# CUG-EMI/HMCMT2D

Measured on NVIDIA B200. Metric: leapfrog_steps_per_sec, higher is better.
Workload: dtype f64 (complex128)

## Files before the change

hmcmt2d_b200/csrc/hmcmt_b200.cu:

```cuda
#include <dlfcn.h>
#include <nccl.h>

#include <algorithm>
#include <cmath>
#include <cstdlib>
#include <cstring>
#include <new>
#include <vector>

#include "../../include/hmcmt_b200.h"
#include "band_factor.cuh"
#include "band_solve.cuh"
#include "mf_solver.cuh"
#include "mt_kernels.cuh"

using namespace hmcmt;

namespace {

template <typename Tp>
struct DevBuf {
    Tp* p = nullptr;
    size_t n = 0;
    int alloc(size_t count) {
// ... 154 lines not shown
        case 14: return launch_factor_T<14>(st, sys, nsys, dom, fwdJobs);
        default: return kErrArg;
    }
}
int launch_solve(cudaStream_t st, int T, const SolveJob* jobs, int njobs, const BandDom& dom) {
    switch (T) {
        case 2: return launch_solve_T<2>(st, jobs, njobs, dom);
        case 4: return launch_solve_T<4>(st, jobs, njobs, dom);
        case 6: return launch_solve_T<6>(st, jobs, njobs, dom);
        case 8: return launch_solve_T<8>(st, jobs, njobs, dom);
        case 10: return launch_solve_T<10>(st, jobs, njobs, dom);
        case 12: return launch_solve_T<12>(st, jobs, njobs, dom);
        case 14: return launch_solve_T<14>(st, jobs, njobs, dom);
        default: return kErrArg;
    }
}
int mf_leaf_size() {
    const char* e = std::getenv("HMCMT_MF_LEAF");
    const int v = e ? std::atoi(e) : 16;
    return v < 1 ? 1 : v;
}
int mf_cross_size() {
    const char* e = std::getenv("HMCMT_MF_CROSS");
    const int v = e ? std::atoi(e) : 0;
    return v < 0 ? 0 : v;
}
int mf_push_size() {
    const char* e = std::getenv("HMCMT_MF_PUSH");
    const int v = e ? std::atoi(e) : 2;
    return v < 0 ? 0 : (v > 7 ? 7 : v);
}
int mf_small_front() {
    const char* e = std::getenv("HMCMT_MF_FSMALL");
    int v = e ? std::atoi(e) : 144;
    return v < 0 ? 0 : (v > 144 ? 144 : v);
}
}

namespace {

void linear_interp(double point, const std::vector<double>& x, int& iL, int& iR, double& wL, double& wR) {
    int n = (int)x.size(), ind = 0;
    double best = std::fabs(point - x[0]);
    for (int i = 1; i < n; ++i) {
        double d = std::fabs(point - x[i]);
        if (d < best) { best = d; ind = i; }
    }
    if (point - x[ind] > 0) { iL = ind; iR = ind + 1; } else { iL = ind - 1; iR = ind; }
    iL = std::max(std::min(iL, n - 1), 0);
    iR = std::max(std::min(iR, n - 1), 0);
    if (iL == iR) { wL = 0.5; wR = 0.5; return; }
    double len = x[iR] - x[iL];
    wL = 1 - (point - x[iL]) / len;
    wR = 1 - (x[iR] - point) / len;
}

__global__ void k_pack_pred(int nData, int nFull, const int* __restrict__ packed2full, const cplx* __restrict__ predFull,
                            cplx* __restrict__ out) {
    int i = blockIdx.x * blockDim.x + threadIdx.x, ch = blockIdx.y;
    if (i < nData) out[(size_t)ch * nData + i] = predFull[(size_t)ch * nFull + packed2full[i]];
}
__global__ void k_pack_pred_real(int nData, int nFull, const int* __restrict__ packed2full, const double* __restrict__ respFull,
                                 double* __restrict__ out) {
    int i = blockIdx.x * blockDim.x + threadIdx.x, ch = blockIdx.y;
    if (i < nData) out[(size_t)ch * nData + i] = respFull[(size_t)ch * 2 * nFull + packed2full[i]];
}
__global__ void k_kick_masked(int nAC, double dt, int kstep, const int* __restrict__ L, const double* __restrict__ grad,
                              double* __restrict__ p) {
// ... 1511 lines not shown
```

hmcmt2d_b200/csrc/mf_kernels.cuh:

```cuda
#pragma once
#include "band_factor.cuh"
#include "mf_solver.cuh"

namespace hmcmt {
namespace mf {

__host__ __device__ __forceinline__ size_t kg_off(int ld, int i, int j, int plane) {
    return ((size_t)((j >> 2) * 2 + plane) * ld + i) * 4 + (j & 3);
}

struct Tables {
    const Front* fronts;
    const int* rows;
    const int* rel;
    const int* children;
    const OrigEntry* orig;
    const Chunk* chunks;
    const int* pos2orig;
    double* fac;
    double* arena[2];
    int64_t facStride, arenaStride[2];
    const cplx* vals;
    int64_t valStride;
    int* status;
// ... 16 lines not shown
    f.re[0] = T[lane]; f.re[1] = T[32 + lane]; f.im[0] = T[64 + lane]; f.im[1] = T[96 + lane];
}
__device__ __forceinline__ void frag_load_t(TileFrag& f, const double* T, int g, int t) {
    const int o0 = tl_off(t, g), o1 = tl_off(4 + t, g);
    f.re[0] = T[o0]; f.re[1] = T[o1]; f.im[0] = T[64 + o0]; f.im[1] = T[64 + o1];
}
__device__ __forceinline__ void frag_store(const TileFrag& f, double* T, int lane) {
    T[lane] = f.re[0]; T[32 + lane] = f.re[1]; T[64 + lane] = f.im[0]; T[96 + lane] = f.im[1];
}
__device__ __forceinline__ void cfrag_load(TileFrag& c, const double* T, int g, int t) {
    const int o = tl_off(g, 2 * t);
    const double2 r = *reinterpret_cast<const double2*>(T + o), i = *reinterpret_cast<const double2*>(T + 64 + o);
    c.re[0] = r.x; c.re[1] = r.y; c.im[0] = i.x; c.im[1] = i.y;
}
__device__ __forceinline__ void cfrag_store(const TileFrag& c, double* T, int g, int t, double sign = 1.0) {
    const int o = tl_off(g, 2 * t);
    *reinterpret_cast<double2*>(T + o) = make_double2(sign * c.re[0], sign * c.re[1]);
    *reinterpret_cast<double2*>(T + 64 + o) = make_double2(sign * c.im[0], sign * c.im[1]);
}
__device__ __forceinline__ void frag_mma(TileFrag& c, TileFrag& x, const TileFrag& a, const TileFrag& b) {
#pragma unroll
    for (int kk = 0; kk < 2; ++kk) {
        dmma884(c.re, a.re[kk], b.re[kk]);
        dmma884(c.im, a.re[kk], b.im[kk]);
        dmma884(x.re, -a.im[kk], b.im[kk]);
        dmma884(x.im, a.im[kk], b.re[kk]);
    }
}
__device__ __forceinline__ void frag_zero(TileFrag& c) { c.re[0] = c.re[1] = c.im[0] = c.im[1] = 0.0; }
__device__ __forceinline__ void frag_add(TileFrag& c, const TileFrag& x) {
    c.re[0] += x.re[0]; c.re[1] += x.re[1]; c.im[0] += x.im[0]; c.im[1] += x.im[1];
}

template <int NW, bool PC = false>
__device__ __forceinline__ void mf_front_factor(double* __restrict__ tiles, double* __restrict__ scratch, double* __restrict__ mbuf,
                                                double* __restrict__ nainv, int* __restrict__ fail, const int nb, const int npb,
                                                const int sReal, unsigned long long* __restrict__ prof = nullptr) {
    const int tid = threadIdx.x, lane = tid & 31;
    long long _s0 = prof ? clock64() : 0;
#define MF_SWEEP_MARK(slot) do { if (prof && tid == 0) { const long long _t = clock64(); atomicAdd(prof + (slot), (unsigned long long)(_t - _s0)); _s0 = _t; } } while (0)
    const int warp = __shfl_sync(0xffffffffu, tid >> 5, 0);
    const int g = lane >> 2, t = lane & 3;
    double* const rawb = scratch;
    double* const mmb = scratch + (size_t)npb * 128;
    for (int kb = 0; kb < npb; ++kb) {
        if (warp == 0) {
            const double* D = mf_tile(tiles, kb, kb);
            auto sym = [&](int r, int c, int pl) { return r >= c ? D[pl * 64 + tl_off(r, c)] : D[pl * 64 + tl_off(c, r)]; };
            cplx a0 = mk(sym(g, 2 * t, 0), sym(g, 2 * t, 1)), a1 = mk(sym(g, 2 * t + 1, 0), sym(g, 2 * t + 1, 1));
            bool bad = false;
            const int left = sReal - 8 * kb;
            gj_invert8<(NW > 4)>(a0, a1, bad, g, t, left < 8 ? (left < 0 ? 0 : left) : 8);
            if (__any_sync(0xffffffffu, bad) && lane == 0) *fail = 1;
            TileFrag p;
            p.re[0] = -a0.x; p.re[1] = -a1.x; p.im[0] = -a0.y; p.im[1] = -a1.y;
            cfrag_store(p, nainv, g, t);
            __syncwarp();
            double* Dw = mf_tile(tiles, kb, kb);
            cfrag_store(p, Dw, g, t);
        }
        if (npb == 1) break;
        __syncthreads();
        MF_SWEEP_MARK(0);
        for (int I = warp; I < npb; I += NW) {
            if (I == kb) continue;
            TileFrag a, b, c, x;
            if (I > kb) frag_load(a, mf_tile(tiles, I, kb), lane);
            else frag_load_t(a, mf_tile(tiles, kb, I), g, t);
            frag_load(b, nainv, lane);
            frag_zero(c); frag_zero(x);
// ... 24 lines not shown
                    TileFrag a, b, c, x;
                    frag_load(a, mmb + (size_t)I * 128, lane);
                    frag_load(b, rawb + (size_t)J * 128, lane);
                    cfrag_load(c, T, g, t);
                    frag_zero(x);
                    frag_mma(c, x, a, b);
                    frag_add(c, x);
                    cfrag_store(c, T, g, t);
                }
                J += NW;
                while (J > I) { J -= I + 1; ++I; }
            }
        }
        __syncthreads();
        MF_SWEEP_MARK(1);
    }
    const int nub = nb - npb;
    if (nub == 0) { __syncthreads(); return; }
    __syncthreads();
    if (npb == 1) MF_SWEEP_MARK(0);
    for (int Iu = warp; Iu < nub; Iu += NW) {
        const int I = npb + Iu;
        for (int kb = 0; kb < npb; ++kb) {
            TileFrag c, x;
            frag_zero(c); frag_zero(x);
            for (int j = 0; j < npb; ++j) {
                TileFrag a, b;
                frag_load(a, mf_tile<PC>(tiles, npb, I, j), lane);
                if (kb >= j) frag_load(b, mf_tile(tiles, kb, j), lane);
                else frag_load_t(b, mf_tile(tiles, j, kb), g, t);
                frag_mma(c, x, a, b);
            }
            frag_add(c, x);
            cfrag_store(c, mbuf + (size_t)(Iu * npb + kb) * 128, g, t);
        }
    }
    __syncthreads();
    MF_SWEEP_MARK(2);
    if (PC) return;
    {
        const int nU = nub * (nub + 1) / 2;
        int I = 0, J = warp;
        while (J > I) { J -= I + 1; ++I; }
        constexpr bool kPair = NW > 4;
        for (int L = warp; L < nU; L += (kPair ? 2 : 1) * NW) {
            const int I0 = I, J0 = J;
            J += NW;
            while (J > I) { J -= I + 1; ++I; }
            const bool two = kPair && L + NW < nU;
            const int I1 = I, J1 = J;
            if (kPair) {
                J += NW;
                while (J > I) { J -= I + 1; ++I; }
            }
            double* T0 = mf_tile(tiles, npb + I0, npb + J0);
            double* T1 = mf_tile(tiles, npb + I1, npb + J1);
            TileFrag c0, x0, c1, x1;
            cfrag_load(c0, T0, g, t);
            frag_zero(x0);
            if (two) { cfrag_load(c1, T1, g, t); frag_zero(x1); }
            for (int kb = 0; kb < npb; ++kb) {
                TileFrag a, b;
                frag_load(a, mbuf + (size_t)(I0 * npb + kb) * 128, lane);
                frag_load(b, mf_tile(tiles, npb + J0, kb), lane);
                frag_mma(c0, x0, a, b);
                if (two) {
                    frag_load(a, mbuf + (size_t)(I1 * npb + kb) * 128, lane);
                    frag_load(b, mf_tile(tiles, npb + J1, kb), lane);
                    frag_mma(c1, x1, a, b);
                }
            }
            frag_add(c0, x0);
            cfrag_store(c0, T0, g, t);
            if (two) { frag_add(c1, x1); cfrag_store(c1, T1, g, t); }
        }
    }
    __syncthreads();
    MF_SWEEP_MARK(3);
#undef MF_SWEEP_MARK
}

template <bool TRANSPOSED>
__device__ __forceinline__ void mf_store_tile(const double* __restrict__ T, double* __restrict__ dst, int ld, int row0, int col0,
                                              double sign, int lane) {
#pragma unroll
    for (int h = 0; h < 2; ++h) {
        const int idx = lane + 32 * h;
        const int chunk = idx >> 4, w = idx & 15, pl = chunk >> 1, cg = chunk & 1, r = w >> 1, c2 = (w & 1) * 2;
        double2 v;
        if (!TRANSPOSED) v = *reinterpret_cast<const double2*>(T + chunk * 32 + w * 2);
        else v = make_double2(T[pl * 64 + tl_off(cg * 4 + c2, r)], T[pl * 64 + tl_off(cg * 4 + c2 + 1, r)]);
        double* out = dst + kg_off(ld, row0 + r, col0 + cg * 4, pl) + c2;
        *reinterpret_cast<double2*>(out) = make_double2(sign * v.x, sign * v.y);
    }
}

template <int NW>
__global__ void __launch_bounds__(NW * 32, NW <= 4 ? (NW == 1 ? 16 : 32 / NW) : (NW == 8 ? 4 : 2))
mf_small_kernel(Tables tb, const SmallDesc* __restrict__ descs) {
    constexpr int NT = NW * 32;
    constexpr bool kMid = NW >= 8;
    extern __shared__ __align__(16) unsigned char mf_smem[];
    SmallDesc& F = *reinterpret_cast<SmallDesc*>(mf_smem);
    const int sys = blockIdx.y, tid = threadIdx.x, lane = tid & 31;
    const int warp = __shfl_sync(0xffffffffu, tid >> 5, 0);
    constexpr int _pc = NW <= 2 ? 0 : (NW == 4 ? 1 : (NW == 8 ? 2 : 3));
    long long _t0 = clock64();
    static_assert(sizeof(SmallDesc) % 4 == 0 && sizeof(SmallDesc) <= kFrontDescBytes, "SmallDesc is copied word by word into the head of the dynamic shared memory");
    for (int i = tid; i < (int)(sizeof(SmallDesc) / 4); i += NT)
        reinterpret_cast<int*>(&F)[i] = reinterpret_cast<const int*>(descs + blockIdx.x)[i];
    __syncthreads();
    const int fp = F.sp + F.up, nb = fp >> 3, npb = F.sp >> 3, nub = nb - npb;
    const int nT = kMid ? mf_pc_row(nb, npb) : nb * (nb + 1) / 2;
    double* tiles = reinterpret_cast<double*>(mf_smem + kFrontDescBytes);
    double* mbuf = tiles + (size_t)nT * 128;
    double* nainv = mbuf + (size_t)(2 * npb > nub * npb ? 2 * npb : nub * npb) * 128;
    int* fail = reinterpret_cast<int*>(nainv + 128);
    int2* relS = reinterpret_cast<int2*>(fail + 4);
    auto rel_parts = [npb](int r) {
        return make_int2((kMid ? mf_pc_row(r >> 3, npb) : (r >> 3) * ((r >> 3) + 1) / 2) * 128 + (r & 7) * 4, (r >> 3) * 128 + ((r & 4) << 3) + (r & 3));
    };
    const int nChild = F.nChild;
    {
        int base = 0;
        for (int c = 0; c < nChild; ++c) {
            const int cu = F.cU[c];
            const int* rel = tb.rel + F.cRel[c];
            for (int i = tid; i < cu; i += NT) relS[base + i] = rel_parts(rel[i]);
            base += cu;
        }
    }
    int* invS = reinterpret_cast<int*>(relS + ((F.cU[0] + F.cU[1] + F.cU[2] + F.cU[3] + 1) & ~1));
    const double* carena = tb.arena[F.par ^ 1] + (size_t)sys * tb.arenaStride[F.par ^ 1];
    constexpr int kBatch = 1;
    struct Batch {
        double2 r01[kBatch], r23[kBatch], i01[kBatch], i23[kBatch];
        int ii[kBatch], jg[kBatch];
        int c;
    };
    int curC = 0, curQ = warp * kBatch;
    auto load_batch = [&](Batch& bt) {
        while (curC < nChild) {
            const int cu = F.cU[curC];
            if (curQ < (((kMid ? F.cPiv[curC] : cu) + 3) >> 2) * ((cu + 31) >> 5)) break;
            ++curC;
            curQ = warp * kBatch;
        }
        bt.c = curC < nChild ? curC : -1;
        if (bt.c < 0) return;
// ... 60 lines not shown
                    if (4 * jg + jj > i || (kMid && 4 * jg + jj >= jEnd)) break;
                    double* d = rowp + relC[4 * jg + jj].y;
                    d[0] += re[jj];
                    d[64] += im[jj];
                }
            }
        };
        for (int c = 0; c < nChild; ++c) {
            while (b0.c == c) {
                scatter(b0);
                b0 = b1;
                load_batch(b1);
            }
            __syncwarp();
            __syncthreads();
        }
        if (nChild == 0) __syncthreads();
    }
    MF_PROF_MARK(2);
    if (tid < F.nOrig) {
        double* d = addr(oe0.lrow, oe0.lcol);
        d[0] += ov0.x;
        d[64] += ov0.y;
    }
    for (int e = tid + NT; e < F.nOrig; e += NT) {
        const OrigEntry oe = tb.orig[F.origPtr + e];
        const cplx v = oe.src < 0 ? mk(1.0, 0.0) : vals[oe.src];
        double* d = addr(oe.lrow, oe.lcol);
        d[0] += v.x;
        d[64] += v.y;
    }
    __syncthreads();
    MF_PROF_MARK(1);
    mf_front_factor<NW, kMid>(tiles, mbuf, mbuf, nainv, fail, nb, npb, F.s, tb.prof ? tb.prof + 32 + _pc * 4 : nullptr);
    if (kMid && nub > 0) {
        const long long tD = tb.prof ? clock64() : 0;
        const int g = lane >> 2, t = lane & 3, up = F.up;
        double* U = tb.arena[F.par] + (size_t)sys * tb.arenaStride[F.par] + F.uOff;
        auto gather = [&](TileFrag& c, int I, int J) {
            const int a = 8 * I + g, b = 8 * J + 2 * t;
            frag_zero(c);
#pragma unroll
            for (int ch = 0; ch < kSmallChildren; ++ch) {
                const int* inv = invS + ch * up;
                const int ia = ch < nChild ? inv[a] : -1;
                if (ia < 0) continue;
                const int ib0 = inv[b], ib1 = inv[b + 1];
                const double* Uc = carena + F.cOff[ch];
                const int ld = F.cLd[ch], off = F.cFirst[ch];
                if (ib0 >= 0 && ib0 <= ia) { c.re[0] += Uc[kg_off(ld, off + ia, off + ib0, 0)]; c.im[0] += Uc[kg_off(ld, off + ia, off + ib0, 1)]; }
                if (ib1 >= 0 && ib1 <= ia) { c.re[1] += Uc[kg_off(ld, off + ia, off + ib1, 0)]; c.im[1] += Uc[kg_off(ld, off + ia, off + ib1, 1)]; }
            }
        };
        auto store = [&](const TileFrag& c, int I, int J) {
            double* o = U + kg_off(up, 8 * I + g, 8 * J + 2 * t, 0);
            *reinterpret_cast<double2*>(o) = make_double2(c.re[0], c.re[1]);
            *reinterpret_cast<double2*>(o + 4 * up) = make_double2(c.im[0], c.im[1]);
        };
        const int nU = nub * (nub + 1) / 2;
        int I = 0, J = warp;
        while (J > I) { J -= I + 1; ++I; }
        for (int L = warp; L < nU; L += 2 * NW) {
            const int I0 = I, J0 = J;
            J += NW;
            while (J > I) { J -= I + 1; ++I; }
            const bool two = L + NW < nU;
            const int I1 = I, J1 = J;
            J += NW;
            while (J > I) { J -= I + 1; ++I; }
            TileFrag c0, x0, c1, x1;
            gather(c0, I0, J0);
            frag_zero(x0);
            if (two) { gather(c1, I1, J1); frag_zero(x1); }
            for (int kb = 0; kb < npb; ++kb) {
                TileFrag a, b;
                frag_load(a, mbuf + (size_t)(I0 * npb + kb) * 128, lane);
                frag_load(b, mf_tile<true>(tiles, npb, npb + J0, kb), lane);
                frag_mma(c0, x0, a, b);
                if (two) {
                    frag_load(a, mbuf + (size_t)(I1 * npb + kb) * 128, lane);
                    frag_load(b, mf_tile<true>(tiles, npb, npb + J1, kb), lane);
                    frag_mma(c1, x1, a, b);
                }
            }
            frag_add(c0, x0);
            store(c0, I0, J0);
            if (two) { frag_add(c1, x1); store(c1, I1, J1); }
        }
        if (tb.prof && tid == 0) atomicAdd(tb.prof + 32 + _pc * 4 + 3, (unsigned long long)(clock64() - tD));
    }
    MF_PROF_MARK(4);
    if (tid == 0 && *fail) tb.status[sys] = kErrSingular;
    double* fac = tb.fac + (size_t)sys * tb.facStride;
    const int sp = F.sp, up = F.up;
    {
        double* G = fac + F.gOff;
        for (int I = warp; I < npb; I += NW)
            for (int J = 0; J < npb; ++J) {
                if (I >= J) mf_store_tile<false>(mf_tile(tiles, I, J), G, sp, I * 8, J * 8, -1.0, lane);
                else mf_store_tile<true>(mf_tile(tiles, J, I), G, sp, I * 8, J * 8, -1.0, lane);
            }
    }
    if (up > 0) {
        double* M = fac + F.mOff;
        for (int I = warp; I < nub; I += NW)
            for (int J = 0; J < npb; ++J) mf_store_tile<false>(mbuf + (size_t)(I * npb + J) * 128, M, up, I * 8, J * 8, -1.0, lane);
    }
    if (!kMid && up > 0) {
        double* U = tb.arena[F.par] + (size_t)sys * tb.arenaStride[F.par] + F.uOff;
        int I = 0, J = warp;
        while (J > I) { J -= I + 1; ++I; }
        for (int L = warp; L < nub * (nub + 1) / 2; L += NW) {
            mf_store_tile<false>(mf_tile(tiles, npb + I, npb + J), U, up, I * 8, J * 8, 1.0, lane);
            J += NW;
            while (J > I) { J -= I + 1; ++I; }
        }
    }
    MF_PROF_MARK(5);
    if (tb.prof && tid == 0) { atomicAdd(tb.prof + _pc * 8 + 6, 1ull); atomicAdd(tb.prof + _pc * 8 + 7, (unsigned long long)npb); }
}

__global__ void mf_asm_orig_kernel(Tables tb, const int2* __restrict__ pairs, int n) {
    const int idx = blockIdx.x * blockDim.x + threadIdx.x, sys = blockIdx.y;
    if (idx >= n) return;
    const int2 pr = pairs[idx];
    const Front& F = tb.fronts[pr.x];
    const OrigEntry oe = tb.orig[pr.y];
    const cplx v = oe.src < 0 ? mk(1.0, 0.0) : tb.vals[(size_t)sys * tb.valStride + oe.src];
    double* A = tb.arena[F.depth & 1] + (size_t)sys * tb.arenaStride[F.depth & 1] + F.frontOff;
    const int fp = F.sp + F.up;
    A[kg_off(fp, oe.lrow, oe.lcol, 0)] += v.x;
    A[kg_off(fp, oe.lrow, oe.lcol, 1)] += v.y;
}
struct AsmTile {
    int front, bi, bj;
    int invPtr;
};
__global__ void __launch_bounds__(256)
mf_asm_gather_kernel(Tables tb, const AsmTile* __restrict__ tilesList, const int* __restrict__ invMaps) {
    const AsmTile at = tilesList[blockIdx.x];
    const int sys = blockIdx.y;
    const Front P = tb.fronts[at.front];
    const int fp = P.sp + P.up, par = P.depth & 1;
    double* A = tb.arena[par] + (size_t)sys * tb.arenaStride[par] + P.frontOff;
    const double* carena = tb.arena[par ^ 1] + (size_t)sys * tb.arenaStride[par ^ 1];
    for (int item = threadIdx.x; item < 64 * 16; item += 256) {
        const int a = at.bi * 64 + (item & 63), b0 = at.bj * 64 + (item >> 6) * 4;
        if (a >= fp || b0 >= ((a >> 3) + 1) * 8) continue;
        double re[4] = {0.0, 0.0, 0.0, 0.0}, im[4] = {0.0, 0.0, 0.0, 0.0};
        for (int c = 0; c < P.nChild; ++c) {
            const int* inv = invMaps + at.invPtr + (size_t)c * fp;
            const int ia = inv[a];
// ... 533 lines not shown
```

hmcmt2d_b200/csrc/mf_solver.cu:

```cuda
#include "mf_solver.cuh"

#include <algorithm>
#include <cstdio>
#include <cstdlib>

#include "mf_kernels.cuh"

namespace hmcmt {
namespace mf {

namespace {
struct PerDeviceOnceMf {
    bool done[64] = {};
    bool need() {
        int dev = 0;
        if (cudaGetDevice(&dev) != cudaSuccess || dev < 0 || dev >= 64) return true;
        if (done[dev]) return false;
        done[dev] = true;
        return true;
    }
};
constexpr size_t kMaxSmem = 227 * 1024;

template <int NW>
int launch_small(cudaStream_t st, const Tables& tb, const SmallDesc* list, int n, int nsys, size_t smem) {
    static PerDeviceOnceMf once;
    if (once.need()) HMCMT_CUDA_TRY(cudaFuncSetAttribute(mf_small_kernel<NW>, cudaFuncAttributeMaxDynamicSharedMemorySize, (int)kMaxSmem));
    mf_small_kernel<NW><<<dim3(n, nsys), NW * 32, smem, st>>>(tb, list);
    return kOk;
}
}

template <typename Tp>
int Solver::upload(const std::vector<Tp>& h, Tp** d) {
    *d = nullptr;
    const size_t n = std::max<size_t>(h.size(), 1);
    if (cudaMalloc(d, n * sizeof(Tp)) != cudaSuccess) return kErrAlloc;
    owned.push_back(*d);
    bytes += n * sizeof(Tp);
    if (!h.empty() && cudaMemcpy(*d, h.data(), h.size() * sizeof(Tp), cudaMemcpyHostToDevice) != cudaSuccess) return kErrCuda;
    return kOk;
}

int Solver::upload_solve_descs(const std::vector<int>& fr, const SolveDesc** d) {
    std::vector<SolveDesc> v;
    v.reserve(fr.size());
    for (int k : fr) {
        const Front& F = S.fronts[k];
        SolveDesc sd{};
        sd.sp = F.sp; sd.up = F.up; sd.s = F.s; sd.u = F.u; sd.cbp = F.cbp; sd.rowPtr = F.rowPtr; sd.updOff = (int)F.updOff;
        sd.nChild = F.nChild;
        sd.gOff = S.chunks[F.chunkPtr].gOff; sd.mOff = S.chunks[F.chunkPtr].mOff;
        for (int c = 0; c < std::min(F.nChild, kDescChildren); ++c) {
            const Front& C = S.fronts[S.children[F.childPtr + c]];
            sd.cRel[c] = C.rowPtr; sd.cUpd[c] = (int)C.updOff; sd.cU[c] = C.u;
        }
        for (int i = 0; i < std::min(F.u, kDescRows); ++i) sd.rows[i] = S.rows[F.rowPtr + i];
        v.push_back(sd);
    }
    SolveDesc* p = nullptr;
    int rc = upload(v, &p);
// ... 41 lines not shown
    MF_TRY(upload(S.orig, &d_orig));
    MF_TRY(upload(S.chunks, &d_chunks));
    MF_TRY(upload(S.pos2orig, &d_pos2orig));
    auto dalloc = [&](void** p, size_t nbytes) {
        *p = nullptr;
        if (nbytes == 0) nbytes = 16;
        if (cudaMalloc(p, nbytes) != cudaSuccess) return (int)kErrAlloc;
        owned.push_back(*p);
        bytes += nbytes;
        return (int)kOk;
    };
    MF_TRY(dalloc((void**)&d_fac, (size_t)nsys * S.factorDoubles * sizeof(double)));
    for (int p = 0; p < 2; ++p) MF_TRY(dalloc((void**)&d_arena[p], (size_t)nsys * S.arenaDoubles[p] * sizeof(double)));
    MF_TRY(dalloc((void**)&d_vals, (size_t)nsys * valCount * sizeof(cplx)));
    MF_TRY(dalloc((void**)&d_v, (size_t)nsys * maxRhs * S.Np * sizeof(cplx)));
    MF_TRY(dalloc((void**)&d_upd, (size_t)nsys * maxRhs * S.updEntries * sizeof(cplx)));
    if (const char* e = std::getenv("HMCMT_MF_PROF"); e && std::atoi(e)) {
        MF_TRY(dalloc((void**)&d_prof, 48 * sizeof(unsigned long long)));
        cudaMemset(d_prof, 0, 48 * sizeof(unsigned long long));
    }

    std::vector<int> invMapsHost;
    const SchedKnobs knobs = SchedKnobs::from_env();
    sched.assign(S.maxDepth + 1, DepthSchedule());
    for (int d = 0; d <= S.maxDepth; ++d) {
        DepthSchedule& D = sched[d];
        const std::vector<int>& sm = S.byDepthSmall[d];
        const std::vector<int>& bg = S.byDepthBig[d];
        int* p = nullptr;
        D.nSmall = (int)sm.size();
        if (D.nSmall) {
            int mx = 0;
            for (int k : sm) mx = std::max(mx, S.fronts[k].fp());
            D.smallWarps = mf_small_warps(mx, knobs);
            D.smallSmem = 0;
            std::vector<SmallDesc> descs;
            for (int k : sm) {
                const Front& F = S.fronts[k];
                D.smallSmem = std::max(D.smallSmem, D.smallWarps >= 8 ? mf_mid_front_smem_bytes(F.fp() / 8, F.sp / 8, mf_rel_total(S, k), F.nChild)
                                                                      : mf_front_smem_bytes(F.fp() / 8, F.sp / 8, mf_rel_total(S, k)));
                SmallDesc sd{};
                sd.sp = F.sp; sd.up = F.up; sd.s = F.s; sd.nChild = F.nChild; sd.nOrig = F.nOrig; sd.origPtr = F.origPtr;
                sd.par = F.depth & 1; sd.front = k;
                sd.gOff = S.chunks[F.chunkPtr].gOff; sd.mOff = S.chunks[F.chunkPtr].mOff; sd.uOff = F.frontOff;
                for (int c = 0; c < std::min(F.nChild, kDescChildren); ++c) {
                    const Front& C = S.fronts[S.children[F.childPtr + c]];
                    sd.cOff[c] = C.frontOff; sd.cLd[c] = C.ldU(); sd.cFirst[c] = C.offU(); sd.cU[c] = C.u; sd.cRel[c] = C.rowPtr;
                    int piv = 0;
                    while (piv < C.u && S.rel[C.rowPtr + piv] < F.sp) ++piv;
                    if (piv > 255) return kErrArg;
                    sd.cPiv[c] = (unsigned char)piv;
                }
                descs.push_back(sd);
            }
            SmallDesc* pd = nullptr;
            MF_TRY(upload(descs, &pd));
            D.smallDescs = pd;
        }
        D.nBig = (int)bg.size();
        D.bigBytes = (size_t)S.bigDoublesAtDepth[d] * sizeof(double);
        std::vector<int> sw, sc(bg);
        for (int k : sm) (mf_solve_by_warp(S.fronts[k]) ? sw : sc).push_back(k);
        D.nSolveWarp = (int)sw.size();
        D.nSolveCta = (int)sc.size();
        if (D.nSolveWarp) MF_TRY(upload_solve_descs(sw, &D.solveWarpList));
        if (D.nSolveCta) { MF_TRY(upload(sc, &p)); D.solveCtaList = p; }
        {
            int mxc = 0;
            for (int k : sc) mxc = std::max(mxc, S.fronts[k].fp());
            D.solveCtaThreads = mf_solve_cta_threads(mxc, knobs);
        }
        if (!D.nBig) continue;
        MF_TRY(upload(bg, &p));
        D.bigList = p;
        std::vector<int2> op;
        int maxChunk = 0;
        for (int k : bg) {
            const Front& F = S.fronts[k];
            for (int e = 0; e < F.nOrig; ++e) op.push_back(make_int2(k, F.origPtr + e));
            maxChunk = std::max(maxChunk, F.nChunk);
        }
        int2* p2 = nullptr;
        D.nOrigPairs = (int)op.size();
        if (D.nOrigPairs) { MF_TRY(upload(op, &p2)); D.origPairs = p2; }
        {
            std::vector<AsmTile> tiles;
            for (int k : bg) {
                const Front& F = S.fronts[k];
// ... 71 lines not shown
#undef MF_TRY
    return kOk;
}

int Solver::set_mt_values(cudaStream_t st, int N, const MtValSys* dSys, int sys0, int n) {
    if (valCount < 3 * (int64_t)N) return kErrArg;
    if (n < 0) n = nsys - sys0;
    if (sys0 < 0 || n < 1 || sys0 + n > nsys) return kErrArg;
    mf_mt_vals_kernel<<<dim3((3 * N + 255) / 256, n), 256, 0, st>>>(N, dSys + sys0, d_vals + (size_t)sys0 * valCount, valCount);
    HMCMT_CUDA_TRY(cudaGetLastError());
    return kOk;
}

int Solver::factor(cudaStream_t st, int* dStatus, int64_t* nLaunches, int sys0, int n) {
    if (n < 0) n = this->nsys - sys0;
    if (sys0 < 0 || n < 1 || sys0 + n > this->nsys) return kErrArg;
    const int nsys = n;
    Tables tb{};
    tb.fronts = d_fronts; tb.rows = d_rows; tb.rel = d_rel; tb.children = d_children; tb.orig = d_orig; tb.chunks = d_chunks;
    tb.pos2orig = d_pos2orig; tb.fac = d_fac + (size_t)sys0 * S.factorDoubles;
    tb.arena[0] = d_arena[0] + (size_t)sys0 * S.arenaDoubles[0]; tb.arena[1] = d_arena[1] + (size_t)sys0 * S.arenaDoubles[1];
    tb.facStride = S.factorDoubles; tb.arenaStride[0] = S.arenaDoubles[0]; tb.arenaStride[1] = S.arenaDoubles[1];
    tb.vals = d_vals + (size_t)sys0 * valCount; tb.valStride = valCount; tb.status = dStatus ? dStatus + sys0 : nullptr; tb.prof = d_prof;
    static PerDeviceOnceMf once;
    if (once.need()) {
        HMCMT_CUDA_TRY(cudaFuncSetAttribute(mf_inv_kernel, cudaFuncAttributeMaxDynamicSharedMemorySize, (int)kMaxSmem));
        HMCMT_CUDA_TRY(cudaFuncSetAttribute(mf_gemm_kernel, cudaFuncAttributeMaxDynamicSharedMemorySize, (int)kGemmSmemBytes));
    }
    int64_t nl = 0;
    for (int d = S.maxDepth; d >= 0; --d) {
        const DepthSchedule& D = sched[d];
        if (D.nSmall) {
            int rc = kOk;
            if (D.smallWarps == 1) rc = launch_small<1>(st, tb, D.smallDescs, D.nSmall, nsys, D.smallSmem);
            else if (D.smallWarps == 2) rc = launch_small<2>(st, tb, D.smallDescs, D.nSmall, nsys, D.smallSmem);
            else if (D.smallWarps == 4) rc = launch_small<4>(st, tb, D.smallDescs, D.nSmall, nsys, D.smallSmem);
            else if (D.smallWarps == 8) rc = launch_small<8>(st, tb, D.smallDescs, D.nSmall, nsys, D.smallSmem);
            else rc = launch_small<16>(st, tb, D.smallDescs, D.nSmall, nsys, D.smallSmem);
            if (rc) return rc;
            ++nl;
        }
        if (!D.nBig) continue;
        if (D.nAsmTiles) {
            mf_asm_gather_kernel<<<dim3(D.nAsmTiles, nsys), 256, 0, st>>>(tb, (const AsmTile*)D.asmTiles, d_invMaps);
            ++nl;
        }
        if (D.nOrigPairs) {
            mf_asm_orig_kernel<<<dim3((D.nOrigPairs + 255) / 256, nsys), 256, 0, st>>>(tb, D.origPairs, D.nOrigPairs);
            ++nl;
        }
        for (size_t c = 0; c < D.chunkSteps.size(); ++c) {
            const DepthSchedule::ChunkStep& cs = D.chunkSteps[c];
            if (!cs.nInv) continue;
            mf_inv_kernel<<<dim3(cs.nInv, nsys), kInvWarps * 32, cs.invSmem, st>>>(tb, cs.invList, (int)c);
            ++nl;
            if (cs.nPanelTiles) {
                mf_gemm_kernel<<<dim3(cs.nPanelTiles, nsys), kGemmThreads, kGemmSmemBytes, st>>>(
                    tb, (const GemmJob*)cs.jobs, (const GemmTile*)cs.panelTiles);
                ++nl;
            }
            if (cs.nSchurTiles) {
                mf_gemm_kernel<<<dim3(cs.nSchurTiles, nsys), kGemmThreads, kGemmSmemBytes, st>>>(
                    tb, (const GemmJob*)cs.jobs, (const GemmTile*)cs.schurTiles);
                ++nl;
            }
        }
    }
// ... 210 lines not shown
```

hmcmt2d_b200/csrc/mf_solver.cuh:

```cuda
#pragma once
#include <cstdint>
#include <vector>

#include "common.cuh"
#include "mf_symbolic.h"

namespace hmcmt {
namespace mf {

struct MtValSys {
    const double* planes;
    double omega;
};

constexpr int kDescChildren = kSmallChildren;
struct SmallDesc {
    int sp, up, s, nChild;
    int nOrig, origPtr, par, front;
    int64_t gOff, mOff, uOff;
    int64_t cOff[kDescChildren];
    int cLd[kDescChildren], cFirst[kDescChildren], cU[kDescChildren], cRel[kDescChildren];
    unsigned char cPiv[kDescChildren];
};

constexpr int kDescRows = 40;
struct SolveDesc {
    int sp, up, s, u;
    int cbp, rowPtr, updOff, nChild;
    int64_t gOff, mOff;
    int cRel[kDescChildren], cUpd[kDescChildren], cU[kDescChildren];
    int rows[kDescRows];
};

struct DepthSchedule {
    int nSmall = 0, smallWarps = 4;
    size_t smallSmem = 0;
    const SmallDesc* smallDescs = nullptr;
    int nBig = 0;
    const int* bigList = nullptr;
    int nOrigPairs = 0;
    const int2* origPairs = nullptr;
    const void* asmTiles = nullptr;
    int nAsmTiles = 0;
    struct ChunkStep {
        const int* invList = nullptr;
        int nInv = 0;
        size_t invSmem = 0;
        const void* jobs = nullptr;
        const void* panelTiles = nullptr;
        int nPanelTiles = 0;
        const void* schurTiles = nullptr;
        int nSchurTiles = 0;
    };
    std::vector<ChunkStep> chunkSteps;
    size_t bigBytes = 0;
    const SolveDesc* solveWarpList = nullptr;
    const int* solveCtaList = nullptr;
    int nSolveWarp = 0, nSolveCta = 0;
    int solveCtaThreads = 256;
};

struct Tables;
struct SolveArgs;

class Solver {
  public:
    static Solver* create(Symbolic&& S, int nsys, int maxRhs, int64_t valCount, int* rc);
    ~Solver();
// ... 59 lines not shown
```

hmcmt2d_b200/csrc/mf_symbolic.h:

```cpp
#pragma once
#include <algorithm>
#include <cstdint>
#include <cstdlib>
#include <functional>
#include <numeric>
#include <queue>
#include <vector>

namespace hmcmt {
namespace mf {

constexpr int kTile = 8;
constexpr int kChunkMax = 96;

inline int pad8(int x) { return (x + 7) & ~7; }

constexpr size_t kFrontDescBytes = 160;
constexpr int kSmallChildren = 4;
inline size_t mf_front_smem_bytes(int nb, int npb, int relTotal = 0) {
    const size_t nT = (size_t)nb * (nb + 1) / 2, nS = 2 * (size_t)npb, nM = (size_t)(nb - npb) * npb;
    return kFrontDescBytes + (nT + (nS > nM ? nS : nM) + 1) * 128 * sizeof(double) + 16 + (((size_t)relTotal + 1) & ~(size_t)1) * 2 * sizeof(int);
}
inline size_t mf_mid_front_smem_bytes(int nb, int npb, int relTotal, int nChild) {
    const size_t nub = (size_t)(nb - npb), nT = (size_t)npb * (npb + 1) / 2 + nub * npb, nS = 2 * (size_t)npb, nM = nub * npb;
    return kFrontDescBytes + (nT + (nS > nM ? nS : nM) + 1) * 128 * sizeof(double) + 16 + (((size_t)relTotal + 1) & ~(size_t)1) * 2 * sizeof(int) +
           (size_t)nChild * nub * 8 * sizeof(int);
}
constexpr size_t kFrontSmemMax = 227 * 1024;

struct Entry {
    int row, col, src;
};

struct OrigEntry {
    int lrow, lcol, src;
};

struct Chunk {
    int p0, p1;
    int64_t gOff, mOff;
};

struct Front {
    int s, sp, u, up;
    int cbp;
    int rowPtr;
    int parent, depth;
    int childPtr, nChild;
    int origPtr, nOrig;
    int chunkPtr, nChunk;
    int isBig;
    int64_t frontOff;
    int64_t updOff;
    int fp() const { return sp + up; }
    int ldU() const { return isBig ? sp + up : up; }
    int offU() const { return isBig ? sp : 0; }
};

struct Symbolic {
    int N = 0, Np = 0, K = 0, maxDepth = 0;
    std::vector<int> pos2orig;
// ... 282 lines not shown
        S.orig.resize(cnt[K]);
        std::vector<int> at(cnt.begin(), cnt.end() - 1);
        for (int k = 0; k < K; ++k) {
            S.fronts[k].origPtr = cnt[k];
            S.fronts[k].nOrig = cnt[k + 1] - cnt[k];
        }
        for (const Entry& e : entries) {
            const int a = S.orig2pos[e.row], b = S.orig2pos[e.col];
            const int lo = std::min(a, b), hi = std::max(a, b);
            const int k = snOf[lo];
            const Front& F = S.fronts[k];
            int lrow;
            if (hi < F.cbp + F.sp) lrow = hi - F.cbp;
            else {
                const int* r0 = S.rows.data() + F.rowPtr;
                const int* it = std::lower_bound(r0, r0 + F.u, hi);
                if (it == r0 + F.u || *it != hi) return false;
                lrow = F.sp + (int)(it - r0);
            }
            S.orig[at[k]++] = OrigEntry{lrow, lo - F.cbp, e.src};
        }
        for (int k = 0; k < K; ++k)
            for (int i = S.fronts[k].s; i < S.fronts[k].sp; ++i) S.orig[at[k]++] = OrigEntry{i, i, -1};
    }
    S.byDepthSmall.assign(S.maxDepth + 1, {});
    S.byDepthBig.assign(S.maxDepth + 1, {});
    int64_t fac = 0, arena[2] = {0, 0}, upd = 0;
    std::vector<int64_t> arenaAtDepth(S.maxDepth + 1, 0);
    for (int k = 0; k < K; ++k) {
        Front& F = S.fronts[k];
        const int fp = F.fp();
        int relTotal = 0;
        for (int c = 0; c < F.nChild; ++c) relTotal += S.fronts[S.children[F.childPtr + c]].u;
        F.isBig = (fp > fSmall || F.nChild > kSmallChildren || mf_front_smem_bytes(fp / 8, F.sp / 8, relTotal) > kFrontSmemMax) ? 1 : 0;
        S.maxFp = std::max(S.maxFp, fp);
        (F.isBig ? S.maxFpBig : S.maxFpSmall) = std::max(F.isBig ? S.maxFpBig : S.maxFpSmall, fp);
        (F.isBig ? S.byDepthBig : S.byDepthSmall)[F.depth].push_back(k);
        F.updOff = upd;
        upd += F.up;
        F.chunkPtr = (int)S.chunks.size();
        const int cmax = F.isBig ? kChunkMax : F.sp;
        for (int p0 = 0; p0 < F.sp; p0 += cmax) {
            const int p1 = std::min(p0 + cmax, F.sp), sc = p1 - p0;
            Chunk c{p0, p1, fac, 0};
            fac += 2 * (int64_t)sc * sc;
            c.mOff = fac;
            fac += 2 * (int64_t)(fp - p1) * sc;
            S.chunks.push_back(c);
            const double a = sc, b = fp - p1;
            S.flops += 8.0 * (0.5 * a * a * a + a * a * b + 0.5 * a * b * b);
        }
        F.nChunk = (int)S.chunks.size() - F.chunkPtr;
    }
    S.bigDoublesAtDepth.assign(S.maxDepth + 1, 0);
    for (int d = 0; d <= S.maxDepth; ++d) {
        for (int k : S.byDepthBig[d]) {
            Front& F = S.fronts[k];
            F.frontOff = arenaAtDepth[d];
            arenaAtDepth[d] += 2 * (int64_t)F.fp() * F.fp();
        }
        S.bigDoublesAtDepth[d] = arenaAtDepth[d];
        for (int k : S.byDepthSmall[d]) {
            Front& F = S.fronts[k];
            F.frontOff = arenaAtDepth[d];
            arenaAtDepth[d] += 2 * (int64_t)F.up * F.up;
        }
    }
    for (int d = 0; d <= S.maxDepth; ++d) arena[d & 1] = std::max(arena[d & 1], arenaAtDepth[d]);
    S.factorDoubles = fac;
    S.arenaDoubles[0] = arena[0];
    S.arenaDoubles[1] = arena[1];
    S.updEntries = upd;
    return true;
}

inline int mf_rel_total(const Symbolic& S, int k) {
    const Front& F = S.fronts[k];
    int n = 0;
    for (int c = 0; c < F.nChild; ++c) n += S.fronts[S.children[F.childPtr + c]].u;
    return n;
}

constexpr int kSolveWarpMaxFp = 64;
constexpr int kSolveMfThreads = 256;

struct SchedKnobs {
    int fp1 = 40, fp2 = 40, fp4 = 64, fp8 = 96;
    int solveThreads = 0;
    static SchedKnobs from_env() {
        auto knob = [](const char* name, int dflt) { const char* e = std::getenv(name); return e ? std::atoi(e) : dflt; };
        SchedKnobs k;
        k.fp1 = knob("HMCMT_MF_FP1", k.fp1); k.fp2 = knob("HMCMT_MF_FP2", k.fp2);
        k.fp4 = knob("HMCMT_MF_FP4", k.fp4); k.fp8 = knob("HMCMT_MF_FP8", k.fp8);
        k.solveThreads = knob("HMCMT_MF_SOLVE_THREADS", 0);
        return k;
    }
};

inline int mf_small_warps(int maxFp, const SchedKnobs& k) {
    return maxFp <= k.fp1 ? 1 : (maxFp <= k.fp2 ? 2 : (maxFp <= k.fp4 ? 4 : (maxFp <= k.fp8 ? 8 : 16)));
}
inline bool mf_solve_by_warp(const Front& F) { return !F.isBig && F.fp() <= kSolveWarpMaxFp && F.nChild <= kSmallChildren; }
inline int mf_solve_cta_threads(int maxFp, const SchedKnobs& k) {
    return k.solveThreads ? k.solveThreads : (maxFp <= 144 ? 128 : kSolveMfThreads);
}

inline bool mf_analyse_csc(int64_t n, const int64_t* rowval, const int64_t* colptr, int leaf, int fSmall, Symbolic& S) {
    std::vector<Entry> ent;
    ent.reserve((size_t)(colptr[n] - 1) / 2 + n);
    std::vector<int> ptr(n + 1, 0);
    for (int64_t j = 0; j < n; ++j)
        for (int64_t k = colptr[j] - 1; k < colptr[j + 1] - 1; ++k) {
            const int64_t i = rowval[k] - 1;
            if (i < 0 || i >= n) return false;
            if (i < j) continue;
            ent.push_back(Entry{(int)i, (int)j, (int)k});
            if (i != j) { ++ptr[i + 1]; ++ptr[j + 1]; }
        }
    for (int64_t i = 0; i < n; ++i) ptr[i + 1] += ptr[i];
    std::vector<int> adj(ptr[n]), at(ptr.begin(), ptr.end() - 1);
    for (const Entry& e : ent)
        if (e.row != e.col) { adj[at[e.row]++] = e.col; adj[at[e.col]++] = e.row; }
    std::vector<std::vector<int>> sn;
    mf_order_graph((int)n, ptr, adj, leaf, sn);
    return mf_symbolic((int)n, sn, ent, fSmall, S);
}

inline void mf_grid_entries(int nl, int nf, std::vector<Entry>& e) {
    const int N = nl * nf;
    e.clear();
    e.reserve((size_t)3 * N);
    for (int l = 0; l < nl; ++l)
        for (int f = 0; f < nf; ++f) {
// ... 10 lines not shown
```

Baseline: 273.0.

## Extend fused small-front kernel to larger fronts by streaming M panel through global

Raises the small-front size cap from 144 to 256. Fronts too large to keep the M' panel in shared memory go to a new 16-warp streaming variant, which writes M' straight to the global factor array and reads it back during the Schur update, computing up to four tiles per row per warp. The goal is to move mid-size fronts off the slower big-front path so they are handled by one fused CTA each. The cost is extra global traffic, one CTA per SM, and a new host check that returns an error if the shared memory limit is exceeded.

```diff
diff --git a/hmcmt2d_b200/csrc/hmcmt_b200.cu b/hmcmt2d_b200/csrc/hmcmt_b200.cu
--- a/hmcmt2d_b200/csrc/hmcmt_b200.cu
+++ b/hmcmt2d_b200/csrc/hmcmt_b200.cu
@@ -210,8 +210,8 @@
 }
 int mf_small_front() {
     const char* e = std::getenv("HMCMT_MF_FSMALL");
-    int v = e ? std::atoi(e) : 144;
-    return v < 0 ? 0 : (v > 144 ? 144 : v);
+    int v = e ? std::atoi(e) : 256;
+    return v < 0 ? 0 : (v > 256 ? 256 : v);
 }
 }
 
diff --git a/hmcmt2d_b200/csrc/mf_kernels.cuh b/hmcmt2d_b200/csrc/mf_kernels.cuh
--- a/hmcmt2d_b200/csrc/mf_kernels.cuh
+++ b/hmcmt2d_b200/csrc/mf_kernels.cuh
@@ -72,10 +72,11 @@
     c.re[0] += x.re[0]; c.re[1] += x.re[1]; c.im[0] += x.im[0]; c.im[1] += x.im[1];
 }
 
-template <int NW, bool PC = false>
+template <int NW, bool PC = false, bool STREAM = false>
 __device__ __forceinline__ void mf_front_factor(double* __restrict__ tiles, double* __restrict__ scratch, double* __restrict__ mbuf,
                                                 double* __restrict__ nainv, int* __restrict__ fail, const int nb, const int npb,
-                                                const int sReal, unsigned long long* __restrict__ prof = nullptr) {
+                                                const int sReal, unsigned long long* __restrict__ prof = nullptr,
+                                                double* mglob = nullptr, const int ldm = 0) {
     const int tid = threadIdx.x, lane = tid & 31;
     long long _s0 = prof ? clock64() : 0;
 #define MF_SWEEP_MARK(slot) do { if (prof && tid == 0) { const long long _t = clock64(); atomicAdd(prof + (slot), (unsigned long long)(_t - _s0)); _s0 = _t; } } while (0)
@@ -166,7 +167,13 @@
                 frag_mma(c, x, a, b);
             }
             frag_add(c, x);
-            cfrag_store(c, mbuf + (size_t)(Iu * npb + kb) * 128, g, t);
+            if (STREAM) {
+                double* o = mglob + kg_off(ldm, 8 * Iu + g, 8 * kb + 2 * t, 0);
+                *reinterpret_cast<double2*>(o) = make_double2(-c.re[0], -c.re[1]);
+                *reinterpret_cast<double2*>(o + 4 * ldm) = make_double2(-c.im[0], -c.im[1]);
+            } else {
+                cfrag_store(c, mbuf + (size_t)(Iu * npb + kb) * 128, g, t);
+            }
         }
     }
     __syncthreads();
@@ -229,11 +236,11 @@
     }
 }
 
-template <int NW>
-__global__ void __launch_bounds__(NW * 32, NW <= 4 ? (NW == 1 ? 16 : 32 / NW) : (NW == 8 ? 4 : 2))
-mf_small_kernel(Tables tb, const SmallDesc* __restrict__ descs) {
+template <int NW, bool STREAM>
+__device__ __forceinline__ void mf_small_front(const Tables& tb, const SmallDesc* __restrict__ descs) {
     constexpr int NT = NW * 32;
     constexpr bool kMid = NW >= 8;
+    static_assert(!STREAM || kMid, "streamed M' exists in the pivot-column layout only");
     extern __shared__ __align__(16) unsigned char mf_smem[];
     SmallDesc& F = *reinterpret_cast<SmallDesc*>(mf_smem);
     const int sys = blockIdx.y, tid = threadIdx.x, lane = tid & 31;
@@ -248,7 +255,7 @@
     const int nT = kMid ? mf_pc_row(nb, npb) : nb * (nb + 1) / 2;
     double* tiles = reinterpret_cast<double*>(mf_smem + kFrontDescBytes);
     double* mbuf = tiles + (size_t)nT * 128;
-    double* nainv = mbuf + (size_t)(2 * npb > nub * npb ? 2 * npb : nub * npb) * 128;
+    double* nainv = mbuf + (size_t)(STREAM || 2 * npb > nub * npb ? 2 * npb : nub * npb) * 128;
     int* fail = reinterpret_cast<int*>(nainv + 128);
     int2* relS = reinterpret_cast<int2*>(fail + 4);
     auto rel_parts = [npb](int r) {
@@ -375,7 +382,9 @@
     }
     __syncthreads();
     MF_PROF_MARK(1);
-    mf_front_factor<NW, kMid>(tiles, mbuf, mbuf, nainv, fail, nb, npb, F.s, tb.prof ? tb.prof + 32 + _pc * 4 : nullptr);
+    double* fac = tb.fac + (size_t)sys * tb.facStride;
+    mf_front_factor<NW, kMid, STREAM>(tiles, mbuf, mbuf, nainv, fail, nb, npb, F.s, tb.prof ? tb.prof + 32 + _pc * 4 : nullptr,
+                                      fac + F.mOff, F.up);
     if (kMid && nub > 0) {
         const long long tD = tb.prof ? clock64() : 0;
         const int g = lane >> 2, t = lane & 3, up = F.up;
@@ -400,41 +409,81 @@
             *reinterpret_cast<double2*>(o) = make_double2(c.re[0], c.re[1]);
             *reinterpret_cast<double2*>(o + 4 * up) = make_double2(c.im[0], c.im[1]);
         };
-        const int nU = nub * (nub + 1) / 2;
-        int I = 0, J = warp;
-        while (J > I) { J -= I + 1; ++I; }
-        for (int L = warp; L < nU; L += 2 * NW) {
-            const int I0 = I, J0 = J;
-            J += NW;
+        if (!STREAM) {
+            const int nU = nub * (nub + 1) / 2;
+            int I = 0, J = warp;
             while (J > I) { J -= I + 1; ++I; }
-            const bool two = L + NW < nU;
-            const int I1 = I, J1 = J;
-            J += NW;
-            while (J > I) { J -= I + 1; ++I; }
-            TileFrag c0, x0, c1, x1;
-            gather(c0, I0, J0);
-            frag_zero(x0);
-            if (two) { gather(c1, I1, J1); frag_zero(x1); }
-            for (int kb = 0; kb < npb; ++kb) {
-                TileFrag a, b;
-                frag_load(a, mbuf + (size_t)(I0 * npb + kb) * 128, lane);
-                frag_load(b, mf_tile<true>(tiles, npb, npb + J0, kb), lane);
-                frag_mma(c0, x0, a, b);
-                if (two) {
-                    frag_load(a, mbuf + (size_t)(I1 * npb + kb) * 128, lane);
-                    frag_load(b, mf_tile<true>(tiles, npb, npb + J1, kb), lane);
-                    frag_mma(c1, x1, a, b);
+            for (int L = warp; L < nU; L += 2 * NW) {
+                const int I0 = I, J0 = J;
+                J += NW;
+                while (J > I) { J -= I + 1; ++I; }
+                const bool two = L + NW < nU;
+                const int I1 = I, J1 = J;
+                J += NW;
+                while (J > I) { J -= I + 1; ++I; }
+                TileFrag c0, x0, c1, x1;
+                gather(c0, I0, J0);
+                frag_zero(x0);
+                if (two) { gather(c1, I1, J1); frag_zero(x1); }
+                for (int kb = 0; kb < npb; ++kb) {
+                    TileFrag a, b;
+                    frag_load(a, mbuf + (size_t)(I0 * npb + kb) * 128, lane);
+                    frag_load(b, mf_tile<true>(tiles, npb, npb + J0, kb), lane);
+                    frag_mma(c0, x0, a, b);
+                    if (two) {
+                        frag_load(a, mbuf + (size_t)(I1 * npb + kb) * 128, lane);
+                        frag_load(b, mf_tile<true>(tiles, npb, npb + J1, kb), lane);
+                        frag_mma(c1, x1, a, b);
+                    }
                 }
-            }
-            frag_add(c0, x0);
-            store(c0, I0, J0);
-            if (two) { frag_add(c1, x1); store(c1, I1, J1); }
+                frag_add(c0, x0);
+                store(c0, I0, J0);
+                if (two) { frag_add(c1, x1); store(c1, I1, J1); }
+            }
+        } else {
+            constexpr int kRow = 4;
+            const double* Mg = fac + F.mOff;
+            auto load_a = [&](TileFrag& a, int I, int kb) {
+#pragma unroll
+                for (int kk = 0; kk < 2; ++kk) {
+                    const double* p = Mg + kg_off(up, 8 * I + g, 8 * kb + 4 * kk + t, 0);
+                    a.re[kk] = -p[0];
+                    a.im[kk] = -p[4 * up];
+                }
+            };
+            int I = 0, q = warp;
+            while (q > I / kRow) { q -= I / kRow + 1; ++I; }
+            while (I < nub) {
+                const int J0 = kRow * q, nJ = min(kRow, I + 1 - J0);
+                TileFrag c[kRow], x[kRow];
+#pragma unroll
+                for (int r = 0; r < kRow; ++r)
+                    if (r < nJ) { gather(c[r], I, J0 + r); frag_zero(x[r]); }
+                TileFrag a;
+                load_a(a, I, 0);
+                for (int kb = 0; kb < npb; ++kb) {
+                    TileFrag an;
+                    if (kb + 1 < npb) load_a(an, I, kb + 1);
+#pragma unroll
+                    for (int r = 0; r < kRow; ++r)
+                        if (r < nJ) {
+                            TileFrag b;
+                            frag_load(b, mf_tile<true>(tiles, npb, npb + J0 + r, kb), lane);
+                            frag_mma(c[r], x[r], a, b);
+                        }
+                    a = an;
+                }
+#pragma unroll
+                for (int r = 0; r < kRow; ++r)
+                    if (r < nJ) { frag_add(c[r], x[r]); store(c[r], I, J0 + r); }
+                q += NW;
+                while (I < nub && q > I / kRow) { q -= I / kRow + 1; ++I; }
+            }
         }
         if (tb.prof && tid == 0) atomicAdd(tb.prof + 32 + _pc * 4 + 3, (unsigned long long)(clock64() - tD));
     }
     MF_PROF_MARK(4);
     if (tid == 0 && *fail) tb.status[sys] = kErrSingular;
-    double* fac = tb.fac + (size_t)sys * tb.facStride;
     const int sp = F.sp, up = F.up;
     {
         double* G = fac + F.gOff;
@@ -444,7 +493,7 @@
                 else mf_store_tile<true>(mf_tile(tiles, J, I), G, sp, I * 8, J * 8, -1.0, lane);
             }
     }
-    if (up > 0) {
+    if (!STREAM && up > 0) {
         double* M = fac + F.mOff;
         for (int I = warp; I < nub; I += NW)
             for (int J = 0; J < npb; ++J) mf_store_tile<false>(mbuf + (size_t)(I * npb + J) * 128, M, up, I * 8, J * 8, -1.0, lane);
@@ -461,6 +510,15 @@
     }
     MF_PROF_MARK(5);
     if (tb.prof && tid == 0) { atomicAdd(tb.prof + _pc * 8 + 6, 1ull); atomicAdd(tb.prof + _pc * 8 + 7, (unsigned long long)npb); }
+}
+
+template <int NW>
+__global__ void __launch_bounds__(NW * 32, NW <= 4 ? (NW == 1 ? 16 : 32 / NW) : (NW == 8 ? 4 : 2))
+mf_small_kernel(Tables tb, const SmallDesc* __restrict__ descs) {
+    mf_small_front<NW, false>(tb, descs);
+}
+__global__ void __launch_bounds__(16 * 32, 1) mf_small_stream_kernel(Tables tb, const SmallDesc* __restrict__ descs) {
+    mf_small_front<16, true>(tb, descs);
 }
 
 __global__ void mf_asm_orig_kernel(Tables tb, const int2* __restrict__ pairs, int n) {
diff --git a/hmcmt2d_b200/csrc/mf_solver.cu b/hmcmt2d_b200/csrc/mf_solver.cu
--- a/hmcmt2d_b200/csrc/mf_solver.cu
+++ b/hmcmt2d_b200/csrc/mf_solver.cu
@@ -27,6 +27,12 @@
     static PerDeviceOnceMf once;
     if (once.need()) HMCMT_CUDA_TRY(cudaFuncSetAttribute(mf_small_kernel<NW>, cudaFuncAttributeMaxDynamicSharedMemorySize, (int)kMaxSmem));
     mf_small_kernel<NW><<<dim3(n, nsys), NW * 32, smem, st>>>(tb, list);
+    return kOk;
+}
+int launch_stream(cudaStream_t st, const Tables& tb, const SmallDesc* list, int n, int nsys, size_t smem) {
+    static PerDeviceOnceMf once;
+    if (once.need()) HMCMT_CUDA_TRY(cudaFuncSetAttribute(mf_small_stream_kernel, cudaFuncAttributeMaxDynamicSharedMemorySize, (int)kMaxSmem));
+    mf_small_stream_kernel<<<dim3(n, nsys), 16 * 32, smem, st>>>(tb, list);
     return kOk;
 }
 }
@@ -134,13 +140,16 @@
         if (D.nSmall) {
             int mx = 0;
             for (int k : sm) mx = std::max(mx, S.fronts[k].fp());
-            D.smallWarps = mf_small_warps(mx, knobs);
+            D.smallStream = mf_small_stream(S, sm);
+            D.smallWarps = D.smallStream ? 16 : mf_small_warps(mx, knobs);
             D.smallSmem = 0;
             std::vector<SmallDesc> descs;
             for (int k : sm) {
                 const Front& F = S.fronts[k];
-                D.smallSmem = std::max(D.smallSmem, D.smallWarps >= 8 ? mf_mid_front_smem_bytes(F.fp() / 8, F.sp / 8, mf_rel_total(S, k), F.nChild)
-                                                                      : mf_front_smem_bytes(F.fp() / 8, F.sp / 8, mf_rel_total(S, k)));
+                const int nb = F.fp() / 8, npb = F.sp / 8, rt = mf_rel_total(S, k);
+                D.smallSmem = std::max(D.smallSmem, D.smallStream ? mf_stream_front_smem_bytes(nb, npb, rt, F.nChild)
+                                                    : D.smallWarps >= 8 ? mf_mid_front_smem_bytes(nb, npb, rt, F.nChild)
+                                                                        : mf_front_smem_bytes(nb, npb, rt));
                 SmallDesc sd{};
                 sd.sp = F.sp; sd.up = F.up; sd.s = F.s; sd.nChild = F.nChild; sd.nOrig = F.nOrig; sd.origPtr = F.origPtr;
                 sd.par = F.depth & 1; sd.front = k;
@@ -156,6 +165,7 @@
                 descs.push_back(sd);
             }
             SmallDesc* pd = nullptr;
+            if (D.smallSmem > kMaxSmem) return kErrArg;
             MF_TRY(upload(descs, &pd));
             D.smallDescs = pd;
         }
@@ -293,7 +303,8 @@
         const DepthSchedule& D = sched[d];
         if (D.nSmall) {
             int rc = kOk;
-            if (D.smallWarps == 1) rc = launch_small<1>(st, tb, D.smallDescs, D.nSmall, nsys, D.smallSmem);
+            if (D.smallStream) rc = launch_stream(st, tb, D.smallDescs, D.nSmall, nsys, D.smallSmem);
+            else if (D.smallWarps == 1) rc = launch_small<1>(st, tb, D.smallDescs, D.nSmall, nsys, D.smallSmem);
             else if (D.smallWarps == 2) rc = launch_small<2>(st, tb, D.smallDescs, D.nSmall, nsys, D.smallSmem);
             else if (D.smallWarps == 4) rc = launch_small<4>(st, tb, D.smallDescs, D.nSmall, nsys, D.smallSmem);
             else if (D.smallWarps == 8) rc = launch_small<8>(st, tb, D.smallDescs, D.nSmall, nsys, D.smallSmem);
diff --git a/hmcmt2d_b200/csrc/mf_solver.cuh b/hmcmt2d_b200/csrc/mf_solver.cuh
--- a/hmcmt2d_b200/csrc/mf_solver.cuh
+++ b/hmcmt2d_b200/csrc/mf_solver.cuh
@@ -34,6 +34,7 @@
 
 struct DepthSchedule {
     int nSmall = 0, smallWarps = 4;
+    bool smallStream = false;
     size_t smallSmem = 0;
     const SmallDesc* smallDescs = nullptr;
     int nBig = 0;
diff --git a/hmcmt2d_b200/csrc/mf_symbolic.h b/hmcmt2d_b200/csrc/mf_symbolic.h
--- a/hmcmt2d_b200/csrc/mf_symbolic.h
+++ b/hmcmt2d_b200/csrc/mf_symbolic.h
@@ -26,7 +26,20 @@
     return kFrontDescBytes + (nT + (nS > nM ? nS : nM) + 1) * 128 * sizeof(double) + 16 + (((size_t)relTotal + 1) & ~(size_t)1) * 2 * sizeof(int) +
            (size_t)nChild * nub * 8 * sizeof(int);
 }
+inline size_t mf_stream_front_smem_bytes(int nb, int npb, int relTotal, int nChild) {
+    const size_t nub = (size_t)(nb - npb), nT = (size_t)npb * (npb + 1) / 2 + nub * npb, nS = 2 * (size_t)npb;
+    return kFrontDescBytes + (nT + nS + 1) * 128 * sizeof(double) + 16 + (((size_t)relTotal + 1) & ~(size_t)1) * 2 * sizeof(int) +
+           (size_t)nChild * nub * 8 * sizeof(int);
+}
 constexpr size_t kFrontSmemMax = 227 * 1024;
+constexpr int kFullFrontMaxFp = 144;
+inline bool mf_front_needs_stream(int nb, int npb, int relTotal, int nChild) {
+    return mf_mid_front_smem_bytes(nb, npb, relTotal, nChild) > kFrontSmemMax;
+}
+inline size_t mf_large_front_smem_bytes(int nb, int npb, int relTotal, int nChild) {
+    return mf_front_needs_stream(nb, npb, relTotal, nChild) ? mf_stream_front_smem_bytes(nb, npb, relTotal, nChild)
+                                                            : mf_mid_front_smem_bytes(nb, npb, relTotal, nChild);
+}
 
 struct Entry {
     int row, col, src;
@@ -375,7 +388,9 @@
         const int fp = F.fp();
         int relTotal = 0;
         for (int c = 0; c < F.nChild; ++c) relTotal += S.fronts[S.children[F.childPtr + c]].u;
-        F.isBig = (fp > fSmall || F.nChild > kSmallChildren || mf_front_smem_bytes(fp / 8, F.sp / 8, relTotal) > kFrontSmemMax) ? 1 : 0;
+        const size_t smem = fp <= kFullFrontMaxFp ? mf_front_smem_bytes(fp / 8, F.sp / 8, relTotal)
+                                                  : mf_large_front_smem_bytes(fp / 8, F.sp / 8, relTotal, F.nChild);
+        F.isBig = (fp > fSmall || F.nChild > kSmallChildren || smem > kFrontSmemMax) ? 1 : 0;
         S.maxFp = std::max(S.maxFp, fp);
         (F.isBig ? S.maxFpBig : S.maxFpSmall) = std::max(F.isBig ? S.maxFpBig : S.maxFpSmall, fp);
         (F.isBig ? S.byDepthBig : S.byDepthSmall)[F.depth].push_back(k);
@@ -441,7 +456,15 @@
 };
 
 inline int mf_small_warps(int maxFp, const SchedKnobs& k) {
-    return maxFp <= k.fp1 ? 1 : (maxFp <= k.fp2 ? 2 : (maxFp <= k.fp4 ? 4 : (maxFp <= k.fp8 ? 8 : 16)));
+    const int w = maxFp <= k.fp1 ? 1 : (maxFp <= k.fp2 ? 2 : (maxFp <= k.fp4 ? 4 : (maxFp <= k.fp8 ? 8 : 16)));
+    return maxFp > kFullFrontMaxFp && w < 8 ? 8 : w;
+}
+inline bool mf_small_stream(const Symbolic& S, const std::vector<int>& launch) {
+    for (int k : launch) {
+        const Front& F = S.fronts[k];
+        if (F.fp() > kFullFrontMaxFp && mf_front_needs_stream(F.fp() / 8, F.sp / 8, mf_rel_total(S, k), F.nChild)) return true;
+    }
+    return false;
 }
 inline bool mf_solve_by_warp(const Front& F) { return !F.isBig && F.fp() <= kSolveWarpMaxFp && F.nChild <= kSmallChildren; }
 inline int mf_solve_cta_threads(int maxFp, const SchedKnobs& k) {
```

Result: faster. 284.9 (median of 6 runs) (+4.4%).
